# davidea97/Fisher-Nerf-customized

Measured on AMD Instinct MI355X. Metric: candidate-views/sec, higher is better.
Workload: dtype f32

## Files before the change

### fisher-nerf-customized_amd/csrc/fisher_rast.hip

```cpp
#include <hip/hip_runtime.h>
#include <hip/hip_fp16.h>
#include <stdint.h>
#include <stdio.h>
#include <stdlib.h>
#include <string.h>
#include "fr_math.h"
#include "../../include/fisher_rast.h"
#include "fr_internal.h"

#define FR_THREADS 256
#define FR_G_MAX 32
#define FR_MAX_LDS_TILES 4096
#define FR_PART_MIN_DEFAULT 2048
#define FR_SORT_SMALL_KEYS 2048
#define FR_SORT_MID_KEYS 4096
#define FR_SORT_BIG_KEYS 16384
#define FR_VC_MAX 16
#define FR_BATCH 256
#define FR_BWD_BATCH 128

#include <vector>
#include <utility>
static thread_local char g_err[512] = "";
#if defined(FR_ABLATE) || defined(FR_LOOPSTATS)
// ... 699 lines not shown
		__syncthreads();
		if (tid == 0) s_np = 0;
		__syncthreads();
	}
	for (int vv = 0; vv < nv; vv++)
	{
		const int v = v0 + vv;
		uint32_t* cnt = p.tile_cnt + (size_t)v * p.T;
		const uint32_t* h = hist + (size_t)vv * p.T;
		for (int t = tid; t < p.T; t += FR_THREADS)
		{
			const uint32_t c = h[t];
			if (c) p.blk_base[((size_t)v * nblk + blockIdx.x) * p.T + t] = atomicAdd(&cnt[t], c);
		}
	}
	if (tid < nv)
	{
		const int v = v0 + tid;
		p.vis_n[(size_t)v * nblk + blockIdx.x] = s_n[tid];
		if (p.vis_count && s_n[tid]) atomicAdd(&p.vis_count[v], (int)s_n[tid]);
		if (p.num_rendered && s_ref[tid]) atomicAdd(&p.num_rendered[v], (int)s_ref[tid]);
	}
	if constexpr (RC != 0 && PHASE_C)
	{
		__syncthreads();
		if (compact)
		{
			for (int t = tid; t < nv * W32; t += FR_THREADS)
			{
				const int vv = t / W32, w = t - vv * W32;
				uint32_t acc = 0;
				for (int u = 0; u < w; u++) acc += (uint32_t)__popc(s_bm[vv * W32 + u]);
				s_pf[t] = acc;
			}
			__syncthreads();
		}
		const size_t PV = (size_t)nblk * cap;
		for (int vv = 0; vv < nv; vv++)
		{
			const int v = v0 + vv;
			const uint32_t n = s_n[vv];
			FrVisEntry* list = p.vis_list + ((size_t)v * nblk + blockIdx.x) * cap;
			float wm[12];
#pragma unroll
			for (int k = 0; k < 12; k++) wm[k] = has_w2c ? s_wm[12 * vv + k] : 0.f;
			for (uint32_t e = tid; e < n; e += FR_THREADS)
			{
				const uint32_t idx = list[e].idx;
				if (compact)
				{
					const uint32_t local = idx - blockIdx.x * cap;
					const uint32_t rank = s_pf[vv * W32 + (int)(local >> 5)] + (uint32_t)__popc(s_bm[vv * W32 + (int)(local >> 5)] & ((1u << (local & 31u)) - 1u));
					const uint32_t slot = blockIdx.x * cap + rank;
					const float4* tmp = (const float4*)(p.splat + ((size_t)v * nblk + blockIdx.x) * cap + e);
					fr_fisher_record_one<(RC < 0 ? -RC : RC), false, (RC < 0)>(p, ra.H_inv, ra.hinv_stride, ra.packed, ra.recq, v, idx, vm, pm, wm, has_w2c,
					                                                           ra.comp + ((size_t)v * PV + slot) * 6, tmp);
					list[e].idx = slot;
					if constexpr (RC < 0) ra.slot_idx[(size_t)v * PV + slot] = idx;
				}
				else fr_fisher_record_one<(RC < 0 ? -RC : RC), false, (RC < 0)>(p, ra.H_inv, ra.hinv_stride, ra.packed, ra.recq, v, idx, vm, pm, wm, has_w2c);
			}
		}
	}
}

template <int C, int AF, bool DK, bool IDV = false, bool SLOTS = false>
__global__ __launch_bounds__(FR_THREADS) void k_preprocess_views_c(FrParams p, FrRecordArgs ra)
{
	static_assert(!SLOTS || (AF == 0 && !IDV), "the slot table is an option of the general score form (the out_H forms always write it)");
	static_assert((C == 4 || C == 11) && AF >= 0 && AF <= 4 && !((AF == 1 || AF >= 3) && C != 4), "records modes: score form, A-form (4 columns), general out_H form, pose form (4 columns), render form (4 columns)");
	static_assert(!IDV || (C == 4 && AF == 0 && DK), "the identity-view front end is the 4-column score form's with fixed key segments");
	constexpr int RS = FrRecStride<C, AF, DK>::value;
	extern __shared__ uint32_t fr_dyn_lds[];
	const int VC = p.VC;
	uint32_t* hist = fr_dyn_lds;
	uint32_t* pairs = hist + (size_t)VC * p.T;
	float* s_wm = (float*)(pairs + FR_THREADS * (VC + 1));
	uint32_t* park = (uint32_t*)(s_wm + 12 * VC);
	__shared__ uint32_t s_n[FR_VC_MAX];
	__shared__ uint32_t s_ref[FR_VC_MAX];
	__shared__ uint32_t s_ca[FR_VC_MAX * 4];
	__shared__ uint32_t s_wk2[2][FR_VC_MAX * 4];
	__shared__ uint32_t s_wtot2[2][4];
	uint32_t batch_no = 0;
	const int tid = threadIdx.x, lane = tid & 63;
	const int wave = __builtin_amdgcn_readfirstlane(tid >> 6);
	const int v0 = blockIdx.y * VC;
	const int nv = min(VC, p.V - v0);
	const uint32_t nblk = gridDim.x;
	const uint32_t cap = (uint32_t)(FR_THREADS * p.G);
	for (int t = tid; t < nv * p.T; t += FR_THREADS) hist[t] = 0;
	const bool has_w2c = p.w2c != nullptr;
	if (has_w2c) for (int t = tid; t < nv * 12; t += FR_THREADS) s_wm[t] = p.w2c[16 * (size_t)(v0 + t / 12) + (t % 12)];
	if (tid < FR_VC_MAX) { s_n[tid] = 0; s_ref[tid] = 0; }
	float vm[16], pm[16];
#pragma unroll
	for (int k = 0; k < 16; k++) { vm[k] = IDV ? (k % 5 == 0 ? 1.f : 0.f) : p.view[k]; pm[k] = p.proj[k]; }
	if constexpr (IDV)
	{
		bool id = true;
#pragma unroll
		for (int k = 0; k < 16; k++) id = id && p.view[k] == vm[k];
		if (!id && tid == 0) { atomicOr(&p.status[1], 1); atomicOr(&p.status[3], 2); }
	}
	const size_t PV = (size_t)nblk * cap;
	const unsigned long long lt = (1ull << lane) - 1ull;
	__syncthreads();
	const int iw = blockIdx.x * p.G * FR_THREADS;
	const bool early = ra.early != 0;
	const float lx = 1.3f * p.tanfovx, ly = 1.3f * p.tanfovy;
	float wn;
	{
		const float c0 = fabsf(vm[0]) + fabsf(vm[1]) + fabsf(vm[2]), c1 = fabsf(vm[4]) + fabsf(vm[5]) + fabsf(vm[6]), c2 = fabsf(vm[8]) + fabsf(vm[9]) + fabsf(vm[10]);
		const float r0 = fabsf(vm[0]) + fabsf(vm[4]) + fabsf(vm[8]), r1 = fabsf(vm[1]) + fabsf(vm[5]) + fabsf(vm[9]), r2 = fabsf(vm[2]) + fabsf(vm[6]) + fabsf(vm[10]);
		wn = fmaxf(c0, fmaxf(c1, c2)) * fmaxf(r0, fmaxf(r1, r2));
	}
	const float fx2 = 1.02f * wn * p.focal_x * p.focal_x, fy2 = 1.02f * wn * p.focal_y * p.focal_y;
	const float xmax = (float)(p.gx * FR_BLOCK_X + FR_BLOCK_X), ymax = (float)(p.gy * FR_BLOCK_Y + FR_BLOCK_Y);
	unsigned long long skipm = 0ull;
	if (early && ra.grp != nullptr && p.G * nv <= 64)
	{
		const float wrow = fabsf(pm[3] - vm[2]) + fabsf(pm[7] - vm[6]) + fabsf(pm[11] - vm[10]) + fabsf(pm[15] - vm[14]);
		const float wmag = fabsf(vm[2]) + fabsf(vm[6]) + fabsf(vm[10]) + fabsf(vm[14]);
		const bool pinhole = wrow <= 1e-6f * wmag;
		bool skip = false;
		const int g = lane / nv, vv = lane - g * nv;
		const int blk = blockIdx.x * p.G + g;
		if (pinhole && g < p.G && blk * FR_THREADS < p.P)
		{
#pragma clang fp contract(fast)
			const float4 b0 = ra.grp[2 * (size_t)blk], b1 = ra.grp[2 * (size_t)blk + 1];
			const fr_f3 cw = { 0.5f * (b0.x + b1.x), 0.5f * (b0.y + b1.y), 0.5f * (b0.z + b1.z) };
			const float ex = b1.x - cw.x, ey = b1.y - cw.y, ez = b1.z - cw.z;
			float R = 1.01f * __builtin_amdgcn_sqrtf(ex * ex + ey * ey + ez * ez) + 1e-6f;
			const fr_f3 c = has_w2c ? fr_world_to_cam(cw, s_wm + 12 * vv) : cw;
			if (has_w2c)
			{
				const float* m = s_wm + 12 * vv;
				const float g00 = m[0] * m[0] + m[4] * m[4] + m[8] * m[8], g11 = m[1] * m[1] + m[5] * m[5] + m[9] * m[9], g22 = m[2] * m[2] + m[6] * m[6] + m[10] * m[10];
				const float g01 = fabsf(m[0] * m[1] + m[4] * m[5] + m[8] * m[9]), g02 = fabsf(m[0] * m[2] + m[4] * m[6] + m[8] * m[10]), g12 = fabsf(m[1] * m[2] + m[5] * m[6] + m[9] * m[10]);
				R *= __builtin_amdgcn_sqrtf(fmaxf(g00 + g01 + g02, fmaxf(g01 + g11 + g12, g02 + g12 + g22))) * 1.00001f;
			}
			const float kcm = fx2 * (1.0f + lx * lx) + fy2 * (1.0f + ly * ly);
			const float a2 = 2.0f * 1.01f * 3.0f * __builtin_amdgcn_sqrtf(kcm * b0.w);
			const float c0 = 6.0f;
			const float Wf = (float)p.W, Hf = (float)p.H;
			const float zc = vm[2] * c.x + vm[6] * c.y + vm[10] * c.z + vm[14];
			const float zn = __builtin_amdgcn_sqrtf(vm[2] * vm[2] + vm[6] * vm[6] + vm[10] * vm[10]);
			auto side = [&](float sx, float sy, float sz, float sw, float kz, float add) -> bool {
				const float Ax = sx + kz * vm[2], Ay = sy + kz * vm[6], Az = sz + kz * vm[10];
				const float Lc = Ax * c.x + Ay * c.y + Az * c.z + (sw + kz * vm[14]) + add;
				return Lc + __builtin_amdgcn_sqrtf(Ax * Ax + Ay * Ay + Az * Az) * R < 0.f;
			};
			const bool left = side(Wf * pm[0], Wf * pm[4], Wf * pm[8], Wf * pm[12], Wf - 1.0f + 2.0f * c0, a2);
			const bool right = side(-Wf * pm[0], -Wf * pm[4], -Wf * pm[8], -Wf * pm[12], -(Wf - 1.0f - 2.0f * xmax - 2.0f * c0), a2);
			const bool top = side(Hf * pm[1], Hf * pm[5], Hf * pm[9], Hf * pm[13], Hf - 1.0f + 2.0f * c0, a2);
			const bool bottom = side(-Hf * pm[1], -Hf * pm[5], -Hf * pm[9], -Hf * pm[13], -(Hf - 1.0f - 2.0f * ymax - 2.0f * c0), a2);
			const bool behind = zc + zn * R <= 0.001f;
			skip = left || right || top || bottom || behind;
		}
		skipm = __builtin_amdgcn_ballot_w64(skip);
	}
	uint32_t pend = 0;
	for (int g = 0; g < p.G; g++)
	{
		const int i0 = iw + g * FR_THREADS;
		if (i0 >= p.P) break;
		const bool last_round = g == p.G - 1 || i0 + FR_THREADS >= p.P;
		uint32_t np = 0;
		const uint32_t skipv = (uint32_t)(skipm >> (g * nv)) & ((1u << nv) - 1u);
		if (skipv != (1u << nv) - 1u)
		{
			const int i = i0 + tid;
			const bool live = i < p.P;
			fr_f3 pw = { 0.f, 0.f, 0.f };
			float tr = 0.f;
			if (live) { const float4 m4 = ra.mt[i]; pw = fr_f3{ m4.x, m4.y, m4.z }; tr = m4.w; }
			uint32_t keepbits = 0;
			for (int vv = 0; vv < nv; vv++)
			{
				if ((skipv >> vv) & 1u) { if (lane == 0) s_ca[vv * 4 + wave] = 0u; continue; }
				const fr_f3 po = has_w2c ? fr_world_to_cam(pw, s_wm + 12 * vv) : pw;
				const fr_f3 p_view = IDV ? po : fr_xform4x3(po, vm);
				bool keep = live && !(p_view.z <= 0.001f);
				if (early)
				{
#pragma clang fp contract(fast)
					const float hx = __builtin_fmaf(pm[8], po.z, __builtin_fmaf(pm[4], po.y, __builtin_fmaf(pm[0], po.x, pm[12])));
					const float hy = __builtin_fmaf(pm[9], po.z, __builtin_fmaf(pm[5], po.y, __builtin_fmaf(pm[1], po.x, pm[13])));
					const float hw = __builtin_fmaf(pm[11], po.z, __builtin_fmaf(pm[7], po.y, __builtin_fmaf(pm[3], po.x, pm[15])));
					const float p_w = __builtin_amdgcn_rcpf(hw + 0.0000001f);
					const float px = ((hx * p_w + 1.0f) * (float)p.W - 1.0f) * 0.5f, py = ((hy * p_w + 1.0f) * (float)p.H - 1.0f) * 0.5f;
					const float iz = __builtin_amdgcn_rcpf(p_view.z);
					const float jx = fminf(fabsf(p_view.x * iz) * 1.001f, lx), jy = fminf(fabsf(p_view.y * iz) * 1.001f, ly);
					const float kc = fx2 * (1.0f + jx * jx) + fy2 * (1.0f + jy * jy);
					const float rb = 3.0f * __builtin_amdgcn_sqrtf(kc * tr * (iz * iz) + 0.7f) * 1.000001f + 2.0f;
					const bool outside = (px + rb < 0.f) || (px - rb > xmax) || (py + rb < 0.f) || (py - rb > ymax);
					keep = keep && !outside;
				}
				keepbits |= (keep ? 1u : 0u) << vv;
				const unsigned long long m = __builtin_amdgcn_ballot_w64(keep);
				if (lane == 0) s_ca[vv * 4 + wave] = (uint32_t)__popcll(m);
			}
			__syncthreads();
			uint32_t cnt_l = lane < 4 * nv ? s_ca[lane] : 0u;
			uint32_t inc = cnt_l;
#pragma unroll
			for (int d = 1; d < 64; d <<= 1)
			{
				const uint32_t y = (uint32_t)__shfl_up((int)inc, d, 64);
				if (lane >= d) inc += y;
			}
			const uint32_t exc = inc - cnt_l;
			np = (uint32_t)__builtin_amdgcn_readlane((int)inc, 63);
			for (int vv = 0; vv < nv; vv++)
			{
				const bool keep = (keepbits >> vv) & 1u;
				const unsigned long long m = __builtin_amdgcn_ballot_w64(keep);
				const uint32_t base = (uint32_t)__builtin_amdgcn_readlane((int)exc, vv * 4 + wave);
				if (keep) pairs[pend + base + (uint32_t)__popcll(m & lt)] = (uint32_t)(g * FR_THREADS + tid) | ((uint32_t)vv << 16);
			}
		}
		__syncthreads();
		FR_ABL(if (p.ablate == 35) np = 0;)
		pend += np;
		const uint32_t ndo = last_round ? pend : (pend & ~(uint32_t)(FR_THREADS - 1));
		for (uint32_t e0 = 0; e0 < ndo; e0 += FR_THREADS)
		{
			const uint32_t e = e0 + (uint32_t)tid;
			const bool active = e < ndo;
			int i = 0, vv = 0;
			fr_splat sp;
			sp.radius = 0;
			float o = 0.f, cg = 0.f;
			uint32_t ext = 0;
			if (active)
			{
					const uint32_t pr = pairs[e];
				i = iw + (int)(pr & 0xffffu);
				vv = (int)(pr >> 16);
				constexpr int PSB = FrPackSize<C>::value;
				const float4* pk = (const float4*)(ra.packed + (size_t)i * PSB);
				const float4 t0 = pk[0], t1 = pk[1], t2 = pk[2];
				const float o_pre = p.opac[p.order ? p.order[i] : (uint32_t)i];
				const fr_f3 pw = fr_f3{ t0.x, t0.y, t0.z };
				float c3[6];
				c3[0] = t0.w; c3[1] = t1.x; c3[2] = t1.y; c3[3] = t1.z; c3[4] = t1.w; c3[5] = t2.x;
				cg = t2.y + t2.z + t2.w;
				float wm[12];
				if (has_w2c)
				{
#pragma unroll
					for (int k = 0; k < 12; k++) wm[k] = s_wm[12 * vv + k];
				}
				const fr_f3 po = has_w2c ? fr_world_to_cam(pw, wm) : pw;
				sp = fr_preprocess_one<IDV>(po, c3, vm, pm, p.W, p.H, p.tanfovx, p.tanfovy, p.focal_x, p.focal_y, p.gx, p.gy);
				if (sp.radius > 0) { o = o_pre; ext = fr_alpha_extent(sp.conx, sp.cony, sp.conz, o); }
				if constexpr (AF == 4) cg = po.z;
			}
			const bool vis = sp.radius > 0;
			uint32_t* s_wk = s_wk2[batch_no & 1u];
			uint32_t* s_wtot = s_wtot2[batch_no & 1u];
			batch_no++;
			const unsigned long long mv = __builtin_amdgcn_ballot_w64(vis);
			if (lane == 0) s_wtot[wave] = (uint32_t)__popcll(mv);
			uint32_t below = 0;
			for (int k = 0; k < nv; k++)
			{
				const unsigned long long mk = __builtin_amdgcn_ballot_w64(vis && vv == k);
				if (lane == 0) s_wk[k * 4 + wave] = (uint32_t)__popcll(mk);
				if (vv == k) below = (uint32_t)__popcll(mk & lt);
			}
			__syncthreads();
			uint32_t rank = 0, pos = 0, nvis = 0;
			{
#pragma unroll
				for (int w = 0; w < 4; w++) { const uint32_t c = s_wtot[w]; nvis += c; pos += (w < wave) ? c : 0u; }
				pos += (uint32_t)__popcll(mv & lt);
			}
			if (vis)
			{
				rank = s_n[vv] + below;
				for (int w = 0; w < wave; w++) rank += s_wk[vv * 4 + w];
			}
			if (vis)
			{
				uint32_t rx0 = sp.rect.x0, rx1 = sp.rect.x1, ry0 = sp.rect.y0, ry1 = sp.rect.y1;
				atomicAdd(&s_ref[vv], (rx1 - rx0) * (ry1 - ry0));
				{
					const float hx = __half2float(__ushort_as_half((unsigned short)(ext & 0xffffu)));
					const float hy = __half2float(__ushort_as_half((unsigned short)(ext >> 16)));
					if (hx < 0.f) { rx1 = rx0; ry1 = ry0; }
					else if (hx < 1e30f)
					{
						const float inv = 1.0f / (float)FR_BLOCK_X;
						const int tx0 = (int)floorf((sp.px - hx) * inv), tx1 = (int)floorf((sp.px + hx) * inv) + 1;
						const int ty0 = (int)floorf((sp.py - hy) * inv), ty1 = (int)floorf((sp.py + hy) * inv) + 1;
						rx0 = (uint32_t)max((int)rx0, tx0); rx1 = (uint32_t)max((int)rx0, min((int)rx1, tx1));
						ry0 = (uint32_t)max((int)ry0, ty0); ry1 = (uint32_t)max((int)ry0, min((int)ry1, ty1));
					}
				}
				uint32_t* h = hist + (size_t)vv * p.T;
				if constexpr (DK)
				{
					const float hx = __half2float(__ushort_as_half((unsigned short)(ext & 0xffffu)));
					const float hy = __half2float(__ushort_as_half((unsigned short)(ext >> 16)));
					ry0 *= 4u; ry1 *= 4u;
					if (hx >= 0.f && hx < 1e30f && rx1 > rx0 && ry1 > ry0)
					{
						const int tx0 = (int)ceilf((sp.px - hx - 15.0f) * 0.0625f), sy0 = (int)ceilf((sp.py - hy - 3.0f) * 0.25f);
						const int sy1 = (int)floorf((sp.py + hy) * 0.25f) + 1;
						rx0 = (uint32_t)max((int)rx0, tx0); rx1 = max(rx0, rx1);
						ry0 = (uint32_t)max((int)ry0, sy0); ry1 = (uint32_t)max((int)ry0, min((int)ry1, sy1));
					}
					if (rx1 > rx0 && ry1 > ry0)
						for (uint32_t y = ry0 >> 2; y <= (ry1 - 1u) >> 2; y++)
							for (uint32_t x = rx0; x < rx1; x++)
								atomicAdd(&h[y * p.gx + x], 1u);
				}
				else
				for (uint32_t y = ry0; y < ry1; y++)
					for (uint32_t x = rx0; x < rx1; x++)
						atomicAdd(&h[y * p.gx + x], 1u);
				park[0 * FR_THREADS + pos] = __float_as_uint(sp.px);
				park[1 * FR_THREADS + pos] = __float_as_uint(sp.py);
				park[2 * FR_THREADS + pos] = ext;
				if constexpr (AF == 4)
				{
					park[3 * FR_THREADS + pos] = __float_as_uint(o);
					park[4 * FR_THREADS + pos] = __float_as_uint(sp.conx);
					park[5 * FR_THREADS + pos] = __float_as_uint(sp.cony);
					park[6 * FR_THREADS + pos] = __float_as_uint(sp.conz);
				}
				else
				{
					park[3 * FR_THREADS + pos] = __float_as_uint(__builtin_amdgcn_logf(o));
					park[4 * FR_THREADS + pos] = __float_as_uint(-0.5f * sp.conx);
					park[5 * FR_THREADS + pos] = __float_as_uint(-sp.cony);
					park[6 * FR_THREADS + pos] = __float_as_uint(-0.5f * sp.conz);
				}
				park[7 * FR_THREADS + pos] = __float_as_uint(cg);
				park[8 * FR_THREADS + pos] = (uint32_t)i;
				park[9 * FR_THREADS + pos] = fr_as_u32(sp.depth);
				park[10 * FR_THREADS + pos] = rx0 | (ry0 << 16);
				park[11 * FR_THREADS + pos] = rx1 | (ry1 << 16);
				park[12 * FR_THREADS + pos] = rank | ((uint32_t)vv << 16);
			}
			__syncthreads();
			if (tid < nv) s_n[tid] += (s_wk[tid * 4] + s_wk[tid * 4 + 1]) + (s_wk[tid * 4 + 2] + s_wk[tid * 4 + 3]);
			FR_ABL(if (p.ablate == 36) nvis = 0;)
			if ((uint32_t)tid < nvis)
			{
					const int r = tid;
				float4 ab[2];
				ab[0] = make_float4(__uint_as_float(park[0 * FR_THREADS + r]), __uint_as_float(park[1 * FR_THREADS + r]),
				                    __uint_as_float(park[2 * FR_THREADS + r]), __uint_as_float(park[3 * FR_THREADS + r]));
				ab[1] = make_float4(__uint_as_float(park[4 * FR_THREADS + r]), __uint_as_float(park[5 * FR_THREADS + r]),
				                    __uint_as_float(park[6 * FR_THREADS + r]), __uint_as_float(park[7 * FR_THREADS + r]));
				const uint32_t idx = park[8 * FR_THREADS + r];
				const uint32_t rk = park[12 * FR_THREADS + r];
				const int cvv = (int)(rk >> 16);
				const uint32_t slot = blockIdx.x * cap + (rk & 0xffffu);
				const int v = v0 + cvv;
				float wm[12];
#pragma unroll
				for (int k = 0; k < 12; k++) wm[k] = has_w2c ? s_wm[12 * cvv + k] : 0.f;
				float4* rec_out = ra.comp + ((size_t)v * PV + slot) * RS;
				FR_ABL(if (p.ablate == 37) rec_out = ra.comp + (size_t)tid * RS;)
				if constexpr (AF == 4)
				{
					const float4 t2 = ((const float4*)(ra.packed + (size_t)idx * FrPackSize<C>::value))[2];
					rec_out[0] = ab[0];
					rec_out[1] = make_float4(ab[1].x, ab[1].y, ab[1].z, __uint_as_float(park[9 * FR_THREADS + r]));
					rec_out[2] = make_float4(t2.y, t2.z, t2.w, ab[1].w);
				}
				else if constexpr (AF >= 2) fr_fisher_record_general<C, (AF == 3)>(p, ra.packed, v, idx, vm, pm, wm, has_w2c, rec_out, ab);
				else fr_fisher_record_one<C, false, (AF == 1), (AF == 0 && DK), IDV>(p, ra.H_inv, ra.hinv_stride, ra.packed, ra.recq, v, idx, vm, pm, wm, has_w2c, rec_out, ab);
				if constexpr (DK)
				{
					const uint32_t xy0 = park[10 * FR_THREADS + r], xy1 = park[11 * FR_THREADS + r];
					const uint32_t rect = (xy0 & 255u) | ((xy0 >> 16) << 8) | (((xy1 & 0xffffu) - (xy0 & 0xffffu)) << 16) | (((xy1 >> 16) - (xy0 >> 16)) << 24);
					((uint2*)p.vis_list)[((size_t)v * nblk + blockIdx.x) * cap + (rk & 0xffffu)] = make_uint2(park[9 * FR_THREADS + r], rect);
				}
				else
				{
					FrVisEntry en;
					en.idx = slot; en.depth_bits = park[9 * FR_THREADS + r];
					en.xy0 = park[10 * FR_THREADS + r]; en.xy1 = park[11 * FR_THREADS + r];
					*(uint4*)(p.vis_list + ((size_t)v * nblk + blockIdx.x) * cap + (rk & 0xffffu)) = *(const uint4*)&en;
				}
				if constexpr (AF == 1 || AF == 2 || SLOTS) ra.slot_idx[(size_t)v * PV + slot] = p.order ? p.order[idx] : idx;
				if constexpr (SLOTS) ra.slot_acc[(size_t)v * PV + slot] = 0.f;
			}
		}
		const uint32_t rem = pend - ndo;
		if (rem != 0u && ndo != 0u)
		{
			uint32_t t = 0;
			if ((uint32_t)tid < rem) t = pairs[ndo + tid];
			__syncthreads();
			if ((uint32_t)tid < rem) pairs[tid] = t;
			__syncthreads();
		}
		pend = rem;
	}
	__syncthreads();
	if constexpr (DK)
	{
		uint32_t* cursor = park + 13 * FR_THREADS;
		uint32_t vend[FR_VC_MAX];
		uint32_t ntot = 0;
#pragma unroll
		for (int k = 0; k < FR_VC_MAX; k++) { if (k < nv) ntot += s_n[k]; vend[k] = ntot; }
		FR_ABL(if (p.ablate == 31) ntot = 0;)
		constexpr int NB = 4;
		uint2 en[NB], nx[NB];
		uint32_t ev[NB], nxv[NB];
		auto load_round = [&](uint32_t e0, uint2 (&de)[NB], uint32_t (&dv)[NB])
		{
#pragma unroll
			for (int b = 0; b < NB; b++)
			{
				const uint32_t e = e0 + b * FR_THREADS + tid;
				uint32_t vv = 0, lo = 0;
#pragma unroll
				for (int k = 0; k < FR_VC_MAX - 1; k++) if (e >= vend[k]) { vv = k + 1; lo = vend[k]; }
				dv[b] = vv;
				de[b] = make_uint2(0u, 0u);
				FR_ABL(if (p.ablate == 33) { if (e < ntot) de[b] = make_uint2(e, (e & 7u) | ((e >> 3 & 15u) << 10) | (2u << 16) | (2u << 24)); } else)
				if (e < ntot) de[b] = ((const uint2*)p.vis_list)[((size_t)(v0 + vv) * nblk + blockIdx.x) * cap + (e - lo)];
			}
		};
		load_round(0u, en, ev);
		const int nb = nv * p.T;
		for (int b0 = 0; b0 < nb; b0 += 4 * FR_THREADS)
		{
			uint32_t c[4], at[4], gt[4];
#pragma unroll
			for (int k = 0; k < 4; k++)
			{
				const int b = b0 + k * FR_THREADS + tid;
				c[k] = b < nb ? hist[b] : 0u;
				gt[k] = (uint32_t)(v0 + b / p.T) * (uint32_t)p.T + (uint32_t)(b % p.T);
			}
#pragma unroll
			for (int k = 0; k < 4; k++)
			{
				at[k] = 0u;
				FR_ABL(if (p.ablate != 34))
				if (c[k]) at[k] = atomicAdd(&p.tile_cnt[gt[k]], c[k]);
			}
#pragma unroll
			for (int k = 0; k < 4; k++)
			{
				const int b = b0 + k * FR_THREADS + tid;
				if (b < nb)
				{
					hist[b] = (c[k] && at[k] + c[k] <= p.tile_cap) ? gt[k] * p.tile_cap + at[k] : 0xffffffffu;
					cursor[b] = 0u;
				}
			}
		}
		__syncthreads();
		for (uint32_t e0 = 0; e0 < ntot; e0 += NB * FR_THREADS)
		{
			const bool more = e0 + NB * FR_THREADS < ntot;
			if (more) load_round(e0 + NB * FR_THREADS, nx, nxv);
#pragma unroll
			for (int b = 0; b < NB; b++)
			{
				const uint32_t e = e0 + b * FR_THREADS + tid;
				const uint32_t lo = ev[b] ? vend[ev[b] - 1] : 0u;
				const uint64_t key = ((uint64_t)en[b].x << 32) | ((blockIdx.x * cap + (e - lo)) << 4);
				const uint32_t r = en[b].y;
				const uint32_t x0 = r & 255u, s0 = (r >> 8) & 255u, x1 = x0 + ((r >> 16) & 255u), s1 = s0 + (r >> 24);
				const uint32_t* hb = hist + (size_t)ev[b] * p.T;
				uint32_t* cu = cursor + (size_t)ev[b] * p.T;
				if (x1 > x0 && s1 > s0)
				for (uint32_t y = s0 >> 2; y <= (s1 - 1u) >> 2; y++)
				{
					const uint32_t a = max(s0, 4u * y) - 4u * y, z = min(s1, 4u * y + 4u) - 4u * y;
					const uint64_t ky = key | (uint64_t)(((1u << z) - 1u) & ~((1u << a) - 1u));
					for (uint32_t x = x0; x < x1; x++)
					{
						const uint32_t t = y * p.gx + x;
						const uint32_t base = hb[t];
						const uint32_t k = atomicAdd(&cu[t], 1u);
						FR_ABL(if (p.ablate != 32 && p.ablate != 33))
						if (base != 0xffffffffu) p.keys[base + k] = ky;
					}
				}
			}
			if (more)
			{
#pragma unroll
				for (int b = 0; b < NB; b++) { en[b] = nx[b]; ev[b] = nxv[b]; }
			}
		}
	}
	else
	{
		for (int vv = 0; vv < nv; vv++)
		{
			const int v = v0 + vv;
			uint32_t* cnt = p.tile_cnt + (size_t)v * p.T;
			const uint32_t* h = hist + (size_t)vv * p.T;
			for (int t = tid; t < p.T; t += FR_THREADS)
			{
				const uint32_t c = h[t];
				if (c) p.blk_base[((size_t)v * nblk + blockIdx.x) * p.T + t] = atomicAdd(&cnt[t], c);
			}
		}
	}
	if (tid < nv)
	{
		const int v = v0 + tid;
		p.vis_n[(size_t)v * nblk + blockIdx.x] = s_n[tid];
		if (p.vis_count && s_n[tid]) atomicAdd(&p.vis_count[v], (int)s_n[tid]);
		if (p.num_rendered && s_ref[tid]) atomicAdd(&p.num_rendered[v], (int)s_ref[tid]);
	}
}
__global__ __launch_bounds__(FR_THREADS) void k_scatter_vis(FrParams p)
{
	extern __shared__ uint32_t fr_dyn_lds[];
	uint32_t* s_cnt = fr_dyn_lds;
	uint32_t* s_base = fr_dyn_lds + p.T;
	if (p.status[1]) return;
	const int tid = threadIdx.x;
	const int v = blockIdx.y;
	const uint32_t nblk = gridDim.x;
	const uint32_t n = p.vis_n[(size_t)v * nblk + blockIdx.x];
	if (n == 0) return;
	const uint32_t* off = p.tile_off + (size_t)v * p.T;
	const uint32_t* bb = p.blk_base + ((size_t)v * nblk + blockIdx.x) * p.T;
	for (int t = tid; t < p.T; t += FR_THREADS) { s_cnt[t] = 0; s_base[t] = off[t] + bb[t]; }
	__syncthreads();
	const uint4* list = (const uint4*)(p.vis_list + ((size_t)v * nblk + blockIdx.x) * (size_t)(FR_THREADS * p.G));
	constexpr int NB = 4;
	for (uint32_t e0 = 0; e0 < n; e0 += NB * FR_THREADS)
	{
		uint4 en[NB];
#pragma unroll
		for (int b = 0; b < NB; b++)
		{
			const uint32_t e = e0 + b * FR_THREADS + tid;
			en[b] = e < n ? list[e] : make_uint4(0u, 0u, 0u, 0u);
		}
#pragma unroll
		for (int b = 0; b < NB; b++)
		{
			const uint64_t key = ((uint64_t)en[b].y << 32) | en[b].x;
			const uint32_t x0 = en[b].z & 0xffffu, y0 = en[b].z >> 16, x1 = en[b].w & 0xffffu, y1 = en[b].w >> 16;
			for (uint32_t y = y0; y < y1; y++)
				for (uint32_t x = x0; x < x1; x++)
				{
					const uint32_t t = y * p.gx + x;
					p.keys[s_base[t] + atomicAdd(&s_cnt[t], 1u)] = key;
				}
		}
	}
// ... 6838 lines not shown
```

### fisher-nerf-customized_amd/csrc/fr_math.h

```cpp
#pragma once
#include <stdint.h>
#include <math.h>
#include <string.h>

#if defined(__HIPCC__)
#define FR_HD __host__ __device__ __forceinline__
#else
#define FR_HD static inline
#endif

#define FR_BLOCK_X 16
#define FR_BLOCK_Y 16

struct fr_f2 { float x, y; };
struct fr_f3 { float x, y, z; };
struct fr_f4 { float x, y, z, w; };

FR_HD uint32_t fr_as_u32(float f) { uint32_t u; memcpy(&u, &f, 4); return u; }
FR_HD float fr_as_f32(uint32_t u) { float f; memcpy(&f, &u, 4); return f; }

FR_HD int fr_f2i(float f)
{
	if (!(f == f)) return 0;
	if (f >= 2147483648.0f) return 2147483647;
// ... 168 lines not shown
	const float J11 = fr_divt<FAST>(focal_y, c.tz);\
	const float J12 = fr_divt<FAST>(-(focal_y * c.ty), (c.tz * c.tz));\
	for (int cc = 0; cc < 3; cc++)\
		for (int r = 0; r < 3; r++)\
			c.Wc[cc][r] = cc == r ? 1.f : 0.f;\
	c.T0[0] = J00; c.T0[1] = 0.f; c.T0[2] = J02;\
	c.T1[0] = 0.f; c.T1[1] = J11; c.T1[2] = J12;\
	for (int i = 0; i < 6; i++) c.c3[i] = cov3D[i];\
	const float c0 = cov3D[0], c1 = cov3D[1], c2 = cov3D[2], c3 = cov3D[3], c4 = cov3D[4], c5 = cov3D[5];\
	const float A00 = J00 * c0 + J02 * c2;\
	const float A20 = J00 * c2 + J02 * c5;\
	const float A01 = J11 * c1 + J12 * c2;\
	const float A11 = J11 * c3 + J12 * c4;\
	const float A21 = J11 * c4 + J12 * c5;\
	c.cov00 = A00 * J00 + A20 * J02;\
	c.cov01 = A01 * J00 + A21 * J02;\
	c.cov11 = A11 * J11 + A21 * J12;
template <bool FAST = false, bool IDV = false>
FR_HD void fr_cov2d_setup(fr_f3 mean, float focal_x, float focal_y, float tan_fovx, float tan_fovy,
                          const float* cov3D, const float* view, fr_cov2d& c)
{
	if constexpr (IDV)
	{
		(void)view;
		if constexpr (FAST) { FR_CONTRACT FR_COV2D_SETUP_ID_BODY }
		else { FR_COV2D_SETUP_ID_BODY }
	}
	else if constexpr (FAST) { FR_CONTRACT FR_COV2D_SETUP_BODY }
	else { FR_COV2D_SETUP_BODY }
}
#undef FR_COV2D_SETUP_BODY
#undef FR_COV2D_SETUP_ID_BODY

struct fr_splat {
	int radius;
	float depth;
	float px, py;
	float conx, cony, conz;
	fr_rect rect;
	uint32_t tiles;
};

template <bool IDV = false>
FR_HD fr_splat fr_preprocess_one(fr_f3 p_orig, const float* cov3D, const float* view, const float* proj,
                                 int W, int H, float tan_fovx, float tan_fovy, float focal_x, float focal_y,
                                 uint32_t gx, uint32_t gy)
{
	fr_splat s;
	s.radius = 0; s.tiles = 0; s.depth = 0.f; s.px = s.py = 0.f; s.conx = s.cony = s.conz = 0.f;
	s.rect.x0 = s.rect.y0 = s.rect.x1 = s.rect.y1 = 0;

	fr_f3 p_view = p_orig;
	if constexpr (!IDV) p_view = fr_xform4x3(p_orig, view);
	if (p_view.z <= 0.001f)
		return s;
	fr_f4 p_hom = fr_xform4x4(p_orig, proj);
	float p_w = 1.0f / (p_hom.w + 0.0000001f);
	float projx = p_hom.x * p_w, projy = p_hom.y * p_w;

	fr_cov2d c;
	fr_cov2d_setup<false, IDV>(p_orig, focal_x, focal_y, tan_fovx, tan_fovy, cov3D, view, c);
	const float covx = c.cov00 + 0.3f, covy = c.cov01, covz = c.cov11 + 0.3f;

	float det = (covx * covz - covy * covy);
	if (det == 0.0f)
		return s;
	float det_inv = 1.f / det;
	float conx = covz * det_inv, cony = -covy * det_inv, conz = covx * det_inv;

	float mid = 0.5f * (covx + covz);
	float lambda1 = mid + sqrtf(fmaxf(0.1f, mid * mid - det));
	float lambda2 = mid - sqrtf(fmaxf(0.1f, mid * mid - det));
	float my_radius = ceilf(3.f * sqrtf(fmaxf(lambda1, lambda2)));
	float px = fr_ndc2pix(projx, W), py = fr_ndc2pix(projy, H);
	int irad = fr_f2i(my_radius);
	fr_rect rc = fr_get_rect(px, py, irad, gx, gy);
	uint32_t tiles = (rc.x1 - rc.x0) * (rc.y1 - rc.y0);
	if (tiles == 0)
		return s;
	s.radius = irad; s.depth = p_view.z; s.px = px; s.py = py;
	s.conx = conx; s.cony = cony; s.conz = conz; s.rect = rc;
	s.tiles = (rc.y1 - rc.y0) * (rc.x1 - rc.x0);
	return s;
}

#define FR_SH_C0 0.28209479177387814f
#define FR_SH_C1 0.4886025119029199f
#define FR_SH_C2_0 1.0925484305920792f
#define FR_SH_C2_1 -1.0925484305920792f
#define FR_SH_C2_2 0.31539156525252005f
#define FR_SH_C2_3 -1.0925484305920792f
#define FR_SH_C2_4 0.5462742152960396f
#define FR_SH_C3_0 -0.5900435899266435f
#define FR_SH_C3_1 2.890611442640554f
#define FR_SH_C3_2 -0.4570457994644658f
#define FR_SH_C3_3 0.3731763325901154f
#define FR_SH_C3_4 -0.4570457994644658f
#define FR_SH_C3_5 1.445305721320277f
#define FR_SH_C3_6 -0.5900435899266435f

FR_HD fr_f3 fr_sh_to_rgb(int deg, fr_f3 pos, fr_f3 campos, const float* sh, uint8_t* clamped3)
{
	fr_f3 dir = { pos.x - campos.x, pos.y - campos.y, pos.z - campos.z };
	const float dx2 = dir.x * dir.x, dy2 = dir.y * dir.y, dz2 = dir.z * dir.z;
	const float len = sqrtf((dx2 + dy2) + dz2);
	dir.x = dir.x / len; dir.y = dir.y / len; dir.z = dir.z / len;
	const float x = dir.x, y = dir.y, z = dir.z;
	float res[3];
	for (int c = 0; c < 3; c++)
	{
#define FR_S(k) sh[3 * (k) + c]
		float result = FR_SH_C0 * FR_S(0);
		if (deg > 0)
		{
			result = result - FR_SH_C1 * y * FR_S(1) + FR_SH_C1 * z * FR_S(2) - FR_SH_C1 * x * FR_S(3);
			if (deg > 1)
			{
				float xx = x * x, yy = y * y, zz = z * z;
				float xy = x * y, yz = y * z, xz = x * z;
				result = result +
					FR_SH_C2_0 * xy * FR_S(4) +
					FR_SH_C2_1 * yz * FR_S(5) +
					FR_SH_C2_2 * (2.0f * zz - xx - yy) * FR_S(6) +
					FR_SH_C2_3 * xz * FR_S(7) +
					FR_SH_C2_4 * (xx - yy) * FR_S(8);
				if (deg > 2)
				{
					result = result +
						FR_SH_C3_0 * y * (3.0f * xx - yy) * FR_S(9) +
						FR_SH_C3_1 * xy * z * FR_S(10) +
						FR_SH_C3_2 * y * (4.0f * zz - xx - yy) * FR_S(11) +
						FR_SH_C3_3 * z * (2.0f * zz - 3.0f * xx - 3.0f * yy) * FR_S(12) +
						FR_SH_C3_4 * x * (4.0f * zz - xx - yy) * FR_S(13) +
						FR_SH_C3_5 * z * (xx - yy) * FR_S(14) +
						FR_SH_C3_6 * x * (xx - 3.0f * yy) * FR_S(15);
				}
			}
		}
#undef FR_S
		result += 0.5f;
		res[c] = result;
	}
	clamped3[0] = (res[0] < 0); clamped3[1] = (res[1] < 0); clamped3[2] = (res[2] < 0);
	fr_f3 out = { fmaxf(res[0], 0.0f), fmaxf(res[1], 0.0f), fmaxf(res[2], 0.0f) };
	return out;
}


#define FR_ABC_BACKWARD_BODY \
	const float limx = 1.3f * tan_fovx; \
	const float limy = 1.3f * tan_fovy; \
	const float x_grad_mul = (c.txtz < -limx || c.txtz > limx) ? 0.f : 1.f; \
	const float y_grad_mul = (c.tytz < -limy || c.tytz > limy) ? 0.f : 1.f; \
	const float* T0 = c.T0; const float* T1 = c.T1; \
	if (nonzero) \
	{ \
		dcov[0] = (T0[0] * T0[0] * dL_da + T0[0] * T1[0] * dL_db + T1[0] * T1[0] * dL_dc); \
		dcov[3] = (T0[1] * T0[1] * dL_da + T0[1] * T1[1] * dL_db + T1[1] * T1[1] * dL_dc); \
		dcov[5] = (T0[2] * T0[2] * dL_da + T0[2] * T1[2] * dL_db + T1[2] * T1[2] * dL_dc); \
		dcov[1] = 2 * T0[0] * T0[1] * dL_da + (T0[0] * T1[1] + T0[1] * T1[0]) * dL_db + 2 * T1[0] * T1[1] * dL_dc; \
		dcov[2] = 2 * T0[0] * T0[2] * dL_da + (T0[0] * T1[2] + T0[2] * T1[0]) * dL_db + 2 * T1[0] * T1[2] * dL_dc; \
		dcov[4] = 2 * T0[2] * T0[1] * dL_da + (T0[1] * T1[2] + T0[2] * T1[1]) * dL_db + 2 * T1[1] * T1[2] * dL_dc; \
	} \
	else \
	{ \
		for (int i = 0; i < 6; i++) dcov[i] = 0; \
// ... 399 lines not shown
```

Before: 48170.

## Precompute per-view world-space cull planes and simplify vis-list view decoding

```diff
diff --git a/fisher-nerf-customized_amd/csrc/fisher_rast.hip b/fisher-nerf-customized_amd/csrc/fisher_rast.hip
--- a/fisher-nerf-customized_amd/csrc/fisher_rast.hip
+++ b/fisher-nerf-customized_amd/csrc/fisher_rast.hip
@@ -805,6 +805,8 @@
 	__shared__ uint32_t s_ca[FR_VC_MAX * 4];
 	__shared__ uint32_t s_wk2[2][FR_VC_MAX * 4];
 	__shared__ uint32_t s_wtot2[2][4];
+	__shared__ __align__(16) float s_pl[FR_VC_MAX * FR_CULL_STRIDE];
+	__shared__ uint32_t s_vend[FR_VC_MAX];
 	uint32_t batch_no = 0;
 	const int tid = threadIdx.x, lane = tid & 63;
 	const int wave = __builtin_amdgcn_readfirstlane(tid >> 6);
@@ -827,25 +829,21 @@
 		if (!id && tid == 0) { atomicOr(&p.status[1], 1); atomicOr(&p.status[3], 2); }
 	}
 	const size_t PV = (size_t)nblk * cap;
-	const unsigned long long lt = (1ull << lane) - 1ull;
+	auto below_lane = [](unsigned long long m) -> uint32_t { return __builtin_amdgcn_mbcnt_hi((uint32_t)(m >> 32), __builtin_amdgcn_mbcnt_lo((uint32_t)m, 0u)); };
 	__syncthreads();
 	const int iw = blockIdx.x * p.G * FR_THREADS;
 	const bool early = ra.early != 0;
 	const float lx = 1.3f * p.tanfovx, ly = 1.3f * p.tanfovy;
-	float wn;
-	{
-		const float c0 = fabsf(vm[0]) + fabsf(vm[1]) + fabsf(vm[2]), c1 = fabsf(vm[4]) + fabsf(vm[5]) + fabsf(vm[6]), c2 = fabsf(vm[8]) + fabsf(vm[9]) + fabsf(vm[10]);
-		const float r0 = fabsf(vm[0]) + fabsf(vm[4]) + fabsf(vm[8]), r1 = fabsf(vm[1]) + fabsf(vm[5]) + fabsf(vm[9]), r2 = fabsf(vm[2]) + fabsf(vm[6]) + fabsf(vm[10]);
-		wn = fmaxf(c0, fmaxf(c1, c2)) * fmaxf(r0, fmaxf(r1, r2));
-	}
+	const float wn = fr_view_norm2(vm);
 	const float fx2 = 1.02f * wn * p.focal_x * p.focal_x, fy2 = 1.02f * wn * p.focal_y * p.focal_y;
 	const float xmax = (float)(p.gx * FR_BLOCK_X + FR_BLOCK_X), ymax = (float)(p.gy * FR_BLOCK_Y + FR_BLOCK_Y);
+	const float kcm = fr_cull_kcmax(fx2, fy2, lx, ly);
+	const bool pinhole = fr_is_pinhole(vm, pm);
+	const bool cull = early && pinhole;
+	if (cull && tid < nv) fr_plane_cull_setup(vm, pm, has_w2c ? s_wm + 12 * tid : nullptr, p.W, p.H, xmax, ymax, s_pl + FR_CULL_STRIDE * tid);
 	unsigned long long skipm = 0ull;
 	if (early && ra.grp != nullptr && p.G * nv <= 64)
 	{
-		const float wrow = fabsf(pm[3] - vm[2]) + fabsf(pm[7] - vm[6]) + fabsf(pm[11] - vm[10]) + fabsf(pm[15] - vm[14]);
-		const float wmag = fabsf(vm[2]) + fabsf(vm[6]) + fabsf(vm[10]) + fabsf(vm[14]);
-		const bool pinhole = wrow <= 1e-6f * wmag;
 		bool skip = false;
 		const int g = lane / nv, vv = lane - g * nv;
 		const int blk = blockIdx.x * p.G + g;
@@ -864,7 +862,6 @@
 				const float g01 = fabsf(m[0] * m[1] + m[4] * m[5] + m[8] * m[9]), g02 = fabsf(m[0] * m[2] + m[4] * m[6] + m[8] * m[10]), g12 = fabsf(m[1] * m[2] + m[5] * m[6] + m[9] * m[10]);
 				R *= __builtin_amdgcn_sqrtf(fmaxf(g00 + g01 + g02, fmaxf(g01 + g11 + g12, g02 + g12 + g22))) * 1.00001f;
 			}
-			const float kcm = fx2 * (1.0f + lx * lx) + fy2 * (1.0f + ly * ly);
 			const float a2 = 2.0f * 1.01f * 3.0f * __builtin_amdgcn_sqrtf(kcm * b0.w);
 			const float c0 = 6.0f;
 			const float Wf = (float)p.W, Hf = (float)p.H;
@@ -884,6 +881,7 @@
 		}
 		skipm = __builtin_amdgcn_ballot_w64(skip);
 	}
+	if (cull) __syncthreads();
 	uint32_t pend = 0;
 	for (int g = 0; g < p.G; g++)
 	{
@@ -900,6 +898,19 @@
 			float tr = 0.f;
 			if (live) { const float4 m4 = ra.mt[i]; pw = fr_f3{ m4.x, m4.y, m4.z }; tr = m4.w; }
 			uint32_t keepbits = 0;
+			if (cull)
+			{
+				const float mag = fr_plane_cull_mag(pw), na2 = fr_plane_cull_na2(kcm, tr);
+				for (int vv = 0; vv < nv; vv++)
+				{
+					if ((skipv >> vv) & 1u) { if (lane == 0) s_ca[vv * 4 + wave] = 0u; continue; }
+					const bool keep = live && !fr_plane_cull_drop(s_pl + FR_CULL_STRIDE * vv, pw, mag, na2);
+					keepbits |= (keep ? 1u : 0u) << vv;
+					const unsigned long long m = __builtin_amdgcn_ballot_w64(keep);
+					if (lane == 0) s_ca[vv * 4 + wave] = (uint32_t)__popcll(m);
+				}
+			}
+			else
 			for (int vv = 0; vv < nv; vv++)
 			{
 				if ((skipv >> vv) & 1u) { if (lane == 0) s_ca[vv * 4 + wave] = 0u; continue; }
@@ -941,7 +952,7 @@
 				const bool keep = (keepbits >> vv) & 1u;
 				const unsigned long long m = __builtin_amdgcn_ballot_w64(keep);
 				const uint32_t base = (uint32_t)__builtin_amdgcn_readlane((int)exc, vv * 4 + wave);
-				if (keep) pairs[pend + base + (uint32_t)__popcll(m & lt)] = (uint32_t)(g * FR_THREADS + tid) | ((uint32_t)vv << 16);
+				if (keep) pairs[pend + base + below_lane(m)] = (uint32_t)(g * FR_THREADS + tid) | ((uint32_t)vv << 16);
 			}
 		}
 		__syncthreads();
@@ -992,14 +1003,14 @@
 			{
 				const unsigned long long mk = __builtin_amdgcn_ballot_w64(vis && vv == k);
 				if (lane == 0) s_wk[k * 4 + wave] = (uint32_t)__popcll(mk);
-				if (vv == k) below = (uint32_t)__popcll(mk & lt);
+				if (vv == k) below = below_lane(mk);
 			}
 			__syncthreads();
 			uint32_t rank = 0, pos = 0, nvis = 0;
 			{
 #pragma unroll
 				for (int w = 0; w < 4; w++) { const uint32_t c = s_wtot[w]; nvis += c; pos += (w < wave) ? c : 0u; }
-				pos += (uint32_t)__popcll(mv & lt);
+				pos += below_lane(mv);
 			}
 			if (vis)
 			{
@@ -1131,10 +1142,15 @@
 	if constexpr (DK)
 	{
 		uint32_t* cursor = park + 13 * FR_THREADS;
-		uint32_t vend[FR_VC_MAX];
-		uint32_t ntot = 0;
-#pragma unroll
-		for (int k = 0; k < FR_VC_MAX; k++) { if (k < nv) ntot += s_n[k]; vend[k] = ntot; }
+		uint32_t ntot = 0, ve0 = 0, ve1 = 0, ve2 = 0;
+		for (int k = 0; k < nv; k++) { ntot += s_n[k]; if (k == 0) ve0 = ntot; if (k == 1) ve1 = ntot; if (k == 2) ve2 = ntot; }
+		if (nv < 3) ve2 = ntot;
+		if (nv < 2) ve1 = ntot;
+		if (nv > 4)
+		{
+			if (tid == 0) { uint32_t a = 0; for (int k = 0; k < nv; k++) { a += s_n[k]; s_vend[k] = a; } }
+			__syncthreads();
+		}
 		FR_ABL(if (p.ablate == 31) ntot = 0;)
 		constexpr int NB = 4;
 		uint2 en[NB], nx[NB];
@@ -1146,9 +1162,18 @@
 			{
 				const uint32_t e = e0 + b * FR_THREADS + tid;
 				uint32_t vv = 0, lo = 0;
-#pragma unroll
-				for (int k = 0; k < FR_VC_MAX - 1; k++) if (e >= vend[k]) { vv = k + 1; lo = vend[k]; }
-				dv[b] = vv;
+				if (nv <= 4)
+				{
+					if (e >= ve0) { vv = 1; lo = ve0; }
+					if (e >= ve1) { vv = 2; lo = ve1; }
+					if (e >= ve2) { vv = 3; lo = ve2; }
+				}
+				else
+				{
+#pragma unroll 1
+					for (int k = 0; k < nv - 1; k++) if (e >= s_vend[k]) { vv = k + 1; lo = s_vend[k]; }
+				}
+				dv[b] = ((e - lo) & 0xffffu) | (vv << 16);
 				de[b] = make_uint2(0u, 0u);
 				FR_ABL(if (p.ablate == 33) { if (e < ntot) de[b] = make_uint2(e, (e & 7u) | ((e >> 3 & 15u) << 10) | (2u << 16) | (2u << 24)); } else)
 				if (e < ntot) de[b] = ((const uint2*)p.vis_list)[((size_t)(v0 + vv) * nblk + blockIdx.x) * cap + (e - lo)];
@@ -1192,13 +1217,11 @@
 #pragma unroll
 			for (int b = 0; b < NB; b++)
 			{
-				const uint32_t e = e0 + b * FR_THREADS + tid;
-				const uint32_t lo = ev[b] ? vend[ev[b] - 1] : 0u;
-				const uint64_t key = ((uint64_t)en[b].x << 32) | ((blockIdx.x * cap + (e - lo)) << 4);
+				const uint64_t key = ((uint64_t)en[b].x << 32) | ((blockIdx.x * cap + (ev[b] & 0xffffu)) << 4);
 				const uint32_t r = en[b].y;
 				const uint32_t x0 = r & 255u, s0 = (r >> 8) & 255u, x1 = x0 + ((r >> 16) & 255u), s1 = s0 + (r >> 24);
-				const uint32_t* hb = hist + (size_t)ev[b] * p.T;
-				uint32_t* cu = cursor + (size_t)ev[b] * p.T;
+				const uint32_t* hb = hist + (size_t)(ev[b] >> 16) * p.T;
+				uint32_t* cu = cursor + (size_t)(ev[b] >> 16) * p.T;
 				if (x1 > x0 && s1 > s0)
 				for (uint32_t y = s0 >> 2; y <= (s1 - 1u) >> 2; y++)
 				{
diff --git a/fisher-nerf-customized_amd/csrc/fr_math.h b/fisher-nerf-customized_amd/csrc/fr_math.h
--- a/fisher-nerf-customized_amd/csrc/fr_math.h
+++ b/fisher-nerf-customized_amd/csrc/fr_math.h
@@ -274,6 +274,77 @@
 	s.conx = conx; s.cony = cony; s.conz = conz; s.rect = rc;
 	s.tiles = (rc.y1 - rc.y0) * (rc.x1 - rc.x0);
 	return s;
+}
+
+#define FR_CULL_STRIDE 24
+
+FR_HD float fr_cull_sqrt(float x)
+{
+#if defined(__HIP_DEVICE_COMPILE__)
+	return __builtin_amdgcn_sqrtf(x);
+#else
+	return sqrtf(x);
+#endif
+}
+FR_HD float fr_view_norm2(const float* vm)
+{
+	const float c0 = fabsf(vm[0]) + fabsf(vm[1]) + fabsf(vm[2]), c1 = fabsf(vm[4]) + fabsf(vm[5]) + fabsf(vm[6]), c2 = fabsf(vm[8]) + fabsf(vm[9]) + fabsf(vm[10]);
+	const float r0 = fabsf(vm[0]) + fabsf(vm[4]) + fabsf(vm[8]), r1 = fabsf(vm[1]) + fabsf(vm[5]) + fabsf(vm[9]), r2 = fabsf(vm[2]) + fabsf(vm[6]) + fabsf(vm[10]);
+	return fmaxf(c0, fmaxf(c1, c2)) * fmaxf(r0, fmaxf(r1, r2));
+}
+FR_HD bool fr_is_pinhole(const float* vm, const float* pm)
+{
+	const float wrow = fabsf(pm[3] - vm[2]) + fabsf(pm[7] - vm[6]) + fabsf(pm[11] - vm[10]) + fabsf(pm[15] - vm[14]);
+	const float wmag = fabsf(vm[2]) + fabsf(vm[6]) + fabsf(vm[10]) + fabsf(vm[14]);
+	return wrow <= 1e-6f * wmag;
+}
+FR_HD float fr_cull_kcmax(float fx2, float fy2, float lx, float ly) { return fx2 * (1.0f + lx * lx) + fy2 * (1.0f + ly * ly); }
+
+FR_HD void fr_plane_cull_setup(const float* vm, const float* pm, const float* w, int W, int H, float xmax, float ymax, float* q)
+{
+	FR_CONTRACT
+	const float c0 = 6.0f, Wf = (float)W, Hf = (float)H;
+	float mmax = 1.0f;
+	if (w) { mmax = 0.f; for (int k = 0; k < 12; k++) mmax = fmaxf(mmax, fabsf(w[k])); }
+	float ems = 0.f;
+#if defined(__HIPCC__)
+#pragma unroll
+#endif
+	for (int k = 0; k < 5; k++)
+	{
+		const int r = k >> 1 & 1;
+		const float sc = k == 0 ? Wf : k == 1 ? -Wf : k == 2 ? Hf : k == 3 ? -Hf : 0.f;
+		const float kz = k == 0 ? Wf - 1.0f + 2.0f * c0 : k == 1 ? -(Wf - 1.0f - 2.0f * xmax - 2.0f * c0)
+		               : k == 2 ? Hf - 1.0f + 2.0f * c0 : k == 3 ? -(Hf - 1.0f - 2.0f * ymax - 2.0f * c0) : 1.0f;
+		float A[4], mg = 0.f;
+		for (int j = 0; j < 4; j++)
+		{
+			const float s = sc * pm[r + 4 * j], z = kz * vm[2 + 4 * j];
+			A[j] = s + z;
+			mg = j < 3 ? mg + (fabsf(s) + fabsf(z)) : mg * mmax + (fabsf(s) + fabsf(z));
+		}
+		for (int j = 0; j < 3; j++) q[4 * k + j] = w ? A[0] * w[j] + A[1] * w[4 + j] + A[2] * w[8 + j] : A[j];
+		q[4 * k + 3] = w ? A[0] * w[3] + A[1] * w[7] + A[2] * w[11] + A[3] : A[3];
+		const float em = 4e-6f * mg;
+		if (k == 4) q[21] = em;
+		else ems = em > ems || em != em ? em : ems;
+	}
+	q[20] = ems;
+	q[22] = q[23] = 0.f;
+}
+FR_HD float fr_plane_cull_mag(fr_f3 p) { return (fabsf(p.x) + fabsf(p.y)) + (fabsf(p.z) + 1.0f); }
+FR_HD float fr_plane_cull_na2(float kcmax, float tr) { return -(2.0f * 1.01f * 3.0f) * fr_cull_sqrt(kcmax * tr); }
+FR_HD bool fr_plane_cull_drop(const float* q, fr_f3 p, float mag, float na2)
+{
+	const float ts = __builtin_fmaf(-q[20], mag, na2), tz = __builtin_fmaf(-q[21], mag, 0.001f);
+	bool d = false;
+#if defined(__HIPCC__)
+#pragma unroll
+#endif
+	for (int k = 0; k < 4; k++)
+		d |= __builtin_fmaf(q[4 * k + 2], p.z, __builtin_fmaf(q[4 * k + 1], p.y, __builtin_fmaf(q[4 * k], p.x, q[4 * k + 3]))) < ts;
+	d |= __builtin_fmaf(q[18], p.z, __builtin_fmaf(q[17], p.y, __builtin_fmaf(q[16], p.x, q[19]))) < tz;
+	return d;
 }
 
 #define FR_SH_C0 0.28209479177387814f
```

Result: no change. 48500, median of 6 (+0.7%).
